# mct10/Speech-Vecalign

Hardware: AMD Instinct MI355X
Metric: aligned doc-pairs/sec (higher is better)
Workload: dtype bf16; 1 GPU; synthetic 4096x4096 d=1024 bf16 embeddings, 4 overlap layers/side, 10 alignment types, band 14, coarse-to-fine (max_size_full_dp=300), 1024 doc-pairs per GPU per step; pipeline=1, N=4096, M=4096, d=1024, overlaps=4, parallelism=dp1 (pairs sharded, no collective)

## Files before the change

### include/svx.h

```cpp
#ifndef SVX_H
#define SVX_H

#include <stdint.h>

#ifdef __cplusplus
extern "C" {
#endif

typedef struct svx_ctx svx_ctx;

enum svx_dtype { SVX_F32 = 0, SVX_F16 = 1, SVX_BF16 = 2 };

enum svx_status {
    SVX_OK = 0,
    SVX_ERR_ARG = 1,
    SVX_ERR_OVERLAPS = 2,
    SVX_ERR_HIP = 3,
    SVX_ERR_TRACEBACK = 4,
    SVX_ERR_NOMEM = 5,
    SVX_ERR_EXTEND = 6,
    SVX_ERR_PATH = 7,
    SVX_ERR_BP = 8
};

// ... 11 lines not shown


int svx_dense_costs(svx_ctx *ctx, const float *vecs0, int k0, int s0, const float *vecs1, int k1, int s1, int d,
                    const float *norm0, const float *norm1, int offset0, int offset1, float *costs);

int svx_dense_dp(svx_ctx *ctx, const float *cost, int s0, int s1, float pen, double *csum, int32_t *bp);

int svx_score_path(svx_ctx *ctx, const int32_t *xx, const int32_t *yy, int64_t n, const float *norm1,
                   const float *norm2, const float *vecs1, int rows1, const float *vecs2, int rows2, int d, float *out);

int svx_sparse_costs(svx_ctx *ctx, const float *vecs0, int k0, int xsize, const float *vecs1, int k1, int ysize,
                     int d, const float *norms0, const float *norms1, const int32_t *path, int A,
                     const int32_t *types_host, int T, int width_over2, float *costs, int32_t *b_offset);

int svx_sparse_dp(svx_ctx *ctx, const float *costs, const int32_t *b_offset_in, int A, int B,
                  const int32_t *types_host, int T, double del_penalty, int x_in_size, int y_in_size,
                  double *csum, int32_t *xp, int32_t *yp, int32_t *b_offset_out);


int svx_make_norm1(svx_ctx *ctx, float *vecs, int64_t rows, int d);

int svx_downsample(svx_ctx *ctx, const float *vecs, int k, int n, int d, float *half);

int svx_compute_norms(svx_ctx *ctx, const float *vecs0, int k0, int n0, const float *vecs1, int k1, int n1, int d,
                      const int32_t *idx, int samples_per_overlap, float *norms0);

int svx_del_penalty(svx_ctx *ctx, const float *scores, int64_t n, double frac, double *del_penalty);

int svx_dense_traceback(svx_ctx *ctx, const int32_t *bp, int s0, int s1, int32_t *align, int32_t *count);

int svx_sparse_traceback(svx_ctx *ctx, const double *csum, const int32_t *xp, const int32_t *yp,
                         const int32_t *b_offset_out, int a_out, int B, int xsize, int ysize, int32_t *align,
                         double *scores, int32_t *count);

int svx_search_path(svx_ctx *ctx, const int32_t *align, const int32_t *n_align, int upsample, int size0,
                    int size1, int32_t *path, int32_t *path_len);

int svx_gather_rows(svx_ctx *ctx, const void *table, int64_t n_rows, int d, int dtype, const int32_t *idx, int64_t n_out,
                    void *out);


int svx_mt19937_choice(uint32_t *key, int32_t *pos, int64_t n, int64_t size, int32_t *out);

int64_t svx_norm_index_count(int n, int m, int k0, int k1, int max_size_full_dp, int num_samps_for_norm, int have_norms0,
                             int have_norms1);
int64_t svx_knob_index_count(int n, int m, int max_size_full_dp, int costs_sample_size);

int svx_draw_indices(uint32_t *key, int32_t *pos, int n, int m, int k0, int k1, int max_size_full_dp, int costs_sample_size,
                     int num_samps_for_norm, int have_norms0, int have_norms1, int32_t *norm_idx, int32_t *knob_idx);

int svx_candidate_table(const char *seg_path, const char *cat_path, const char *ignore_path, int max_overlaps, int32_t *table,
                        int cap_lines, int32_t *n_lines, int64_t *n_candidates, char *err, int err_cap);

int64_t svx_format_alignments(const int32_t *rows, const double *scores, int64_t n, char *out, int64_t cap);


#define SVX_MARGIN_RATIO 0
#define SVX_MARGIN_DISTANCE 1
#define SVX_MARGIN_ABSOLUTE 2

int svx_unit_rows(svx_ctx *ctx, const void *rows, int dtype, int64_t n, int d, void *out, int out_dtype);

int svx_knn_mean_sim(svx_ctx *ctx, const void *queries, int q_dtype, int64_t n, const void *db, int db_dtype,
                     int64_t n_db, int d, int k, float *mean_sim);

int svx_knn_topk_merge(svx_ctx *ctx, const void *queries, int q_dtype, int64_t n, const void *db, int db_dtype,
// ... 130 lines not shown
```

### speech-vecalign_amd/csrc/svx_api.hip

```cpp
#include <stdarg.h>
#include <stdio.h>
#include <stdlib.h>
#include <string.h>

#include <chrono>
#include <functional>
#include <memory>
#include <type_traits>
#include <vector>

#include "svx_common.h"

static char g_err[512] = "";

int svx_fail(svx_ctx* ctx, int code, const char* fmt, ...) {
    char* dst = ctx ? ctx->err : g_err;
    va_list ap;
    va_start(ap, fmt);
    vsnprintf(dst, 512, fmt, ap);
    va_end(ap);
    return code;
}

static const char* kStageNames[] = {"pyr0",       "pyrN",     "pyr_aux",      "knob_scoresN", "knob",      "dense_costs",
// ... 435 lines not shown
    float* part = reinterpret_cast<float*>(ctx->arena + o_part);
    float* mean = reinterpret_cast<float*>(ctx->arena + o_mean);
    if ((rc = svxl_pairsum(ctx, vecs, k, n, d, half, part, nblk))) return rc;
    if ((rc = svxl_colmean_plain(ctx, part, k, nblk, d, h, mean))) return rc;
    return svxl_sub_mean(ctx, half, k, h, d, mean);
}

int svx_compute_norms(svx_ctx* ctx, const float* vecs0, int k0, int n0, const float* vecs1, int k1, int n1, int d,
                      const int32_t* idx, int samples_per_overlap, float* norms0) {
    NEED(ctx, ctx && vecs0 && vecs1 && idx && norms0, "svx_compute_norms: null argument");
    NEED(ctx, n1 > 0 && samples_per_overlap > 0 && k1 > 0, "svx_compute_norms: nothing to sample");
    int rc = check_dim(ctx, d);
    if (rc) return rc;
    rc = arena_reserve(ctx, (size_t)d * sizeof(float) + 256);
    if (rc) return rc;
    float* rbar = reinterpret_cast<float*>(ctx->arena);
    if ((rc = svxl_sample_mean_plain(ctx, vecs1, k1, n1, d, idx, samples_per_overlap, rbar))) return rc;
    return svxl_norms_from_rbar(ctx, vecs0, (int64_t)k0 * n0, d, rbar, norms0);
}

int svx_del_penalty(svx_ctx* ctx, const float* scores, int64_t n, double frac, double* del_penalty) {
    NEED(ctx, ctx && scores && del_penalty && n > 0, "svx_del_penalty: null/empty argument");
    return svxl_del_penalty(ctx, scores, n, frac, del_penalty);
}

int svx_dense_traceback(svx_ctx* ctx, const int32_t* bp, int s0, int s1, int32_t* align, int32_t* count) {
    NEED(ctx, ctx && bp && align && count, "svx_dense_traceback: null argument");
    return svxl_dense_traceback(ctx, bp, s0, s1, align, count);
}

int svx_sparse_traceback(svx_ctx* ctx, const double* csum, const int32_t* xp, const int32_t* yp, const int32_t* b_offset_out,
                         int a_out, int B, int xsize, int ysize, int32_t* align, double* scores, int32_t* count) {
    NEED(ctx, ctx && csum && xp && yp && b_offset_out && align && scores && count, "svx_sparse_traceback: null argument");
    return svxl_sparse_traceback(ctx, csum, xp, yp, b_offset_out, a_out, B, xsize, ysize, align, scores, count);
}

int svx_search_path(svx_ctx* ctx, const int32_t* align, const int32_t* n_align, int upsample, int size0, int size1,
                    int32_t* path, int32_t* path_len) {
    NEED(ctx, ctx && align && n_align && path && path_len, "svx_search_path: null argument");
    return svxl_search_path(ctx, align, n_align, upsample, size0, size1, path, size0 + size1 + 4, path_len);
}

int svx_gather_rows(svx_ctx* ctx, const void* table, int64_t n_rows, int d, int dtype, const int32_t* idx, int64_t n_out, void* out) {
    NEED(ctx, ctx && table && idx && out, "svx_gather_rows: null argument");
    NEED(ctx, dtype == SVX_F32 || dtype == SVX_F16 || dtype == SVX_BF16, "svx_gather_rows: unknown dtype %d", dtype);
    int rc = check_dim(ctx, d);
    if (rc) return rc;
    return svxl_gather_rows(ctx, table, n_rows, d * (dtype == SVX_F32 ? 4 : 2), dtype, idx, n_out, out);
}

}

__global__ void k_init_batch(const SvxPairDev* pairs) {
    const SvxPairDev& P = pairs[blockIdx.x];
    if (threadIdx.x != 0) return;
    *P.status = 0;
    for (int l = 0; l <= P.L; l++) {
        if (P.lev[l].n_align) *P.lev[l].n_align = 0;
        if (P.lev[l].path_len) *P.lev[l].path_len = 0;
    }
    if (P.straight) {
        int* r = P.lev[0].align;
        r[0] = 0; r[1] = P.lev[0].n[0]; r[2] = 0; r[3] = P.lev[0].n[1];
        *P.lev[0].n_align = 1;
    }
}

// ... 421 lines not shown
    cur.lb.push_back({(np * (H.maxL + 1) * 0.21 < 300.0 ? 300.0 : np * (H.maxL + 1) * 0.21), S_KNOB,
                      [=]() { return svxl_del_penalty_batch(ctx, h->dpairs, np, h->maxL + 1, bp.frac); }});
    if (!bp.straight)
        cur.lb.push_back({(H.max_ds0 + H.max_ds1) * 1.7 * waves, S_DENSE_DP, [=]() { return svxl_dense_stage_batch(ctx, h->dpairs, np, h->max_ds0); }});
    const int first_depth = H.maxL > 0 ? H.maxL - 1 : 0;
    for (int depth = first_depth; depth >= 0; depth--) {
        const SvxTypes ty = depth == 0 ? bp.tfinal : bp.t11;
        int lim2 = 0, tamax2 = 0;
        const bool v2 = !bp.tiles && svxl_band2_limits(ty, W, depth, dtype, d, &lim2, &tamax2);
        const int maxA = H.max_A[depth];
        const int src_rows = (H.maxL > 0 && !H.any_L0) ? maxA / 2 + 8 : maxA;
        cur.lb.push_back({maxA * 0.08 * waves + 60.0, depth == 0 ? S_PATH0 : S_PATH, [=]() {
            return svxl_search_path_batch(ctx, h->dpairs, np, depth, maxA, src_rows, v2 ? lim2 : SVX_BC_ROWS - SVX_BC_TB,
                                          bp.tiles ? 0 : (v2 ? tamax2 : SVX_BC_TAMAX));
        }});
        cur.has_s = true;
        if (bp.tiles) {
            cur.s = {1.0e4, S_TILES, [=]() {
                int* tk = reinterpret_cast<int*>(h->arena + h->o_tickets);
                float* planes = h->b_planes ? reinterpret_cast<float*>(h->arena + h->o_planes) : nullptr;
                return svxl_band_tiles_batch(ctx, h->dpairs, np, ty, W, dtype, h->max_tnd, tk, tk + (size_t)h->max_tnd * np + 1, planes);
            }};
        } else {
            cur.s = {H.b_bc[depth] / 4.0e6, depth == 0 ? S_BAND_COSTS0 : S_BAND_COSTSN, [=]() {
                return v2 ? svxl_band_costs2_batch(ctx, h->dpairs, np, depth, maxA, ty, W, dtype, d)
                          : svxl_band_costs_batch(ctx, h->dpairs, np, depth, maxA, ty, W, dtype, d);
            }};
        }
        segs.push_back(cur);
        cur = Seg();
        if (!bp.tiles)
            cur.lb.push_back({maxA * (0.21 + 0.054 * (ty.n > 1 ? ty.n : 0)) * waves, depth == 0 ? S_BAND_DP0 : S_BAND_DPN,
                              [=]() { return svxl_sparse_dp_batch(ctx, h->dpairs, np, depth, ty, B); }});
        cur.lb.push_back({maxA * 0.27 * waves, depth == 0 ? S_TRACEBACK0 : S_TRACEBACK, [=]() { return svxl_sparse_traceback_batch(ctx, h->dpairs, np, depth, B, maxA, bp.packable ? 1 : 0); }});
    }
    segs.push_back(cur);
}

static int ensure_streams(svx_ctx* ctx) {
    svx_ctx_ext* cx = X(ctx);
    if (!cx->side_ready) {
        int prio_lo = 0, prio_hi = 0;
        SVX_HIP(ctx, hipDeviceGetStreamPriorityRange(&prio_lo, &prio_hi));
        SVX_HIP(ctx, hipStreamCreateWithPriority(&cx->side, hipStreamNonBlocking, prio_lo));
        SVX_HIP(ctx, hipStreamCreateWithPriority(&cx->helper, hipStreamNonBlocking, prio_hi));
        SVX_HIP(ctx, hipEventCreateWithFlags(&cx->side_fork, hipEventDisableTiming));
        SVX_HIP(ctx, hipEventCreateWithFlags(&cx->side_join, hipEventDisableTiming));
        cx->side_ready = true;
    }
    if (!cx->chain_ready) {
        int prio_lo = 0, prio_hi = 0;
        SVX_HIP(ctx, hipDeviceGetStreamPriorityRange(&prio_lo, &prio_hi));
        SVX_HIP(ctx, hipStreamCreateWithPriority(&cx->chain, hipStreamNonBlocking, prio_hi));
        cx->chain_ready = true;
    }
    for (int h = 0; h < 2; h++) {
        if (!cx->half[h].front_done) SVX_HIP(ctx, hipEventCreateWithFlags(&cx->half[h].front_done, hipEventDisableTiming));
        if (!cx->half[h].chain_done) SVX_HIP(ctx, hipEventCreateWithFlags(&cx->half[h].chain_done, hipEventDisableTiming));
        if (!cx->half[h].upload_done) SVX_HIP(ctx, hipEventCreateWithFlags(&cx->half[h].upload_done, hipEventDisableTiming));
    }
    return SVX_OK;
}

static int run_interleaved(svx_ctx* ctx, HalfState* front, HalfState* chain, bool beside) {
    svx_ctx_ext* cx = X(ctx);
    hipStream_t A = ctx->stream, Bst = beside ? cx->chain : ctx->stream;
    std::vector<Op> fops;
// ... 204 lines not shown
```

### speech-vecalign_amd/csrc/svx_common.h

```cpp
#pragma once
#include <hip/hip_runtime.h>
#include <stdint.h>
#include <stddef.h>
#include "../../include/svx.h"

#define SVX_WAVE 64

#ifndef SVX_PYR_SLOTS
#define SVX_PYR_SLOTS 32
#endif
#define SVX_BC_TA 32
#define SVX_BC_TAMAX 64
#define SVX_BC_TB 16
#define SVX_BC_ROWS 48

struct ElemF32 {
    using storage = float;
    static constexpr int VEC = 4;
    static constexpr int DT = SVX_F32;
};
struct ElemF16 {
    using storage = uint16_t;
    static constexpr int VEC = 8;
    static constexpr int DT = SVX_F16;
// ... 234 lines not shown
int svxl_sub_mean(svx_ctx*, float* half, int k, int h, int d, const float* mean);
int svxl_sample_mean_plain(svx_ctx*, const float* vecs, int k, int n, int d, const int* idx, int S, float* rbar);
int svxl_norms_from_rbar(svx_ctx*, const float* vecs, int64_t rows, int d, const float* rbar, float* norms);
int svxl_gather_rows(svx_ctx*, const void* table, long long n_rows, int row_bytes, int dtype, const int* idx, long long n_out, void* out);
int svxl_pyramid_level(svx_ctx*, const SvxPairDev* pairs, int n_pairs, int level, int dtype, int d, int max_nblk,
                       int max_ksum, int part);
int svxl_score_path(svx_ctx*, const int* xx, const int* yy, int64_t n, const float* n1, const float* n2,
                    const float* v1, int rows1, const float* v2, int rows2, int d, float* out);
int svxl_knob_scores(svx_ctx*, const SvxPairDev* pairs, int n_pairs, int max_levels, int max_kn, int max_n0, int dtype, int d,
                     int part);
int svxl_dense_costs(svx_ctx*, const float* v0, int s0, const float* v1, int s1, int d, const float* n0,
                     const float* n1, int mul0, int mul1, float* costs);
int svxl_dense_costs_batch(svx_ctx*, const SvxPairDev* pairs, int n_pairs, int max_s0, int max_s1, int dtype, int d);
int svxl_knob_from_dots(svx_ctx*, const SvxPairDev* pairs, int n_pairs, int max_kn);
int svxl_band_costs(svx_ctx*, const void* v0, int k0, int n, const void* v1, int k1, int m, int d, int dtype,
                    const float* inv0, const float* inv1, const float* nrm0, const float* nrm1, const int* path,
                    int A, const SvxTypes& types, int W, float* costs, int* boff, int* status);
int svxl_band_costs_batch(svx_ctx*, const SvxPairDev* pairs, int n_pairs, int depth, int max_A, const SvxTypes& types,
                          int W, int dtype, int d);
bool svxl_band2_limits(const SvxTypes& types, int W, int depth, int dtype, int d, int* lim, int* tamax);
int svxl_band_costs2_batch(svx_ctx*, const SvxPairDev* pairs, int n_pairs, int depth, int max_A, const SvxTypes& types, int W,
                           int dtype, int d);
int svxl_band_tiles_shape(const SvxTypes& types);
size_t svxl_band_tiles_scratch(const SvxTypes& types);
int svxl_band_tiles_batch(svx_ctx*, const SvxPairDev* pairs, int n_pairs, const SvxTypes& types, int W, int dtype, int max_nd,
                          int* gpref, int* ticket, float* planes);
int svxl_dense_dp(svx_ctx*, const float* cost, int s0, int s1, float pen, double* csum, int* bp);
int svxl_dense_stage_batch(svx_ctx*, const SvxPairDev* pairs, int n_pairs, int max_s0);
int svxl_dense_traceback(svx_ctx*, const int* bp, int s0, int s1, int* align, int* count);
int svxl_sparse_dp(svx_ctx*, const float* costs, const int* boff_in, int A, int B, const SvxTypes& types, double pen,
                   int xs, int ys, double* csum, int* xp, int* yp, int* boff_out);
int svxl_sparse_dp_batch(svx_ctx*, const SvxPairDev* pairs, int n_pairs, int depth, const SvxTypes& types, int B);
int svxl_sparse_traceback(svx_ctx*, const double* csum, const int* xp, const int* yp, const int* boff, int a_out,
                          int B, int xs, int ys, int* align, double* scores, int* count);
int svxl_sparse_traceback_batch(svx_ctx*, const SvxPairDev* pairs, int n_pairs, int depth, int B, int max_A, int packed);
int svxl_search_path(svx_ctx*, const int* align, const int* n_align, int upsample, int size0, int size1, int* path,
                     int cap, int* path_len);
int svxl_search_path_batch(svx_ctx*, const SvxPairDev* pairs, int n_pairs, int depth, int max_rows, int max_src_rows, int chunk_lim,
                           int chunk_tamax);
int svxl_del_penalty(svx_ctx*, const float* scores, int64_t n, double frac, double* out);
int svxl_del_penalty_batch(svx_ctx*, const SvxPairDev* pairs, int n_pairs, int max_levels, double frac);
int svxl_prior_ingest_batch(svx_ctx*, const SvxPairDev* pairs, int n_pairs);
bool svxl_last_batch(svx_ctx*, const SvxPairDev** host, int* n_pairs, int* band);
```

### speech-vecalign_amd/csrc/svx_dp.hip

```cpp
#include <stdlib.h>

#include "svx_common.h"

namespace {

struct DenseDpArgs {
    const float* cost;
    int s0, s1;
    float pen;
    double* csum;
    int* bp;
    int diag;
};

__device__ void dense_dp_block(const DenseDpArgs& g, double* ring) {
    const int rmax = g.s0 + 1, cmax = g.s1 + 1;
    const int tid = threadIdx.x, nt = blockDim.x;
    const double pen_d = (double)g.pen;
    auto cost_of = [&](int k, int r) -> float {
        const int c = k - r;
        return (r >= 1 && r <= g.s0 && c >= 1 && c <= g.s1) ? g.cost[(size_t)(r - 1) * g.s1 + (c - 1)] : 0.f;
    };
    float cnext = cost_of(0, tid);
    for (int k = 0; k <= g.s0 + g.s1; k++) {
// ... 531 lines not shown
}

template <bool RING>
__global__ __launch_bounds__(1024) void k_sparse_dp_batch(const SvxPairDev* __restrict__ pairs, int depth, SvxTypes ty, int B) {
    extern __shared__ __attribute__((aligned(16))) char smem[];
    SparseDpArgs g;
    if (!batch_dp_args(pairs[blockIdx.x], depth, B, &g)) return;
    const size_t ring_bytes = RING ? (((size_t)(ty.maxstep + 1) * g.B * sizeof(double) + 15) & ~(size_t)15) : 0;
    sparse_dp_block<RING>(g, ty, reinterpret_cast<double*>(smem), reinterpret_cast<int*>(smem + ring_bytes));
}

template <int TPLT, int G>
__global__ __launch_bounds__(DPF_THREADS) void k_sparse_dp_fast_batch(const SvxPairDev* __restrict__ pairs, int depth,
                                                                       SvxTypes ty, int B, int CH) {
    extern __shared__ __attribute__((aligned(16))) char smem[];
    SparseDpArgs g;
    if (!batch_dp_args(pairs[blockIdx.x], depth, B, &g)) return;
    sparse_dp_fast<TPLT, G>(g, ty, CH, smem);
}

struct TbArgs {
    const double* csum;
    const int* xp;
    const int* yp;
    const unsigned char* bpk;
    const int* boff;
    int Aout, B, xs, ys;
    int* align;
    double* scores;
    int* count;
    int* status;
    int chunk;
    int cw;
};

__host__ __device__ inline size_t tb_win_bytes(int chunk, int B, bool wide) {
    const size_t bp = (size_t)chunk * B * (wide ? 2 : 1);
    return ((bp + 15) & ~(size_t)15) + (size_t)chunk * sizeof(int);
}
constexpr int TB_COR_CHUNK = 64, TB_COR_W = 320;
__host__ __device__ inline size_t tb_smem_bytes(int chunk, int B, bool wide) { return 2 * tb_win_bytes(chunk, B, wide); }
__host__ __device__ inline int tb_chunk(int B, bool wide, int win_kb = 20) {
    const int c = (int)(((size_t)win_kb * 1024) / ((size_t)B * (wide ? 2 : 1) + sizeof(int))) & ~15;
    if (c >= 64) return c;
    const int c20 = (int)((20 * 1024) / ((size_t)B * (wide ? 2 : 1) + sizeof(int))) & ~15;
    return c20 >= 64 ? c20 : 0;
}
static int tb_win_kb() {
    static const int v = [] { const char* e = getenv("SVX_TB_WIN_KB"); const int k = e ? atoi(e) : 20; return k >= 2 && k <= 64 ? k : 20; }();
    return v;
}

__device__ __forceinline__ void tb_load_corridor(const TbArgs& g, char* win, int j, int c0, int tsub, int nsub) {
    const int lo = j * g.chunk;
    const int hi = (lo + g.chunk) < g.Aout ? (lo + g.chunk) : g.Aout;
    int* lbo = reinterpret_cast<int*>(win + ((((size_t)g.chunk * g.cw) + 15) & ~(size_t)15));
    for (int i = tsub; i < hi - lo; i += nsub) lbo[i] = g.boff[lo + i];
    const int ppr = g.cw / 16;
    const int n = (hi - lo) * ppr;
    for (int e = tsub; e < n; e += nsub) {
        const int i = e / ppr, p = e - i * ppr;
        reinterpret_cast<uint4*>(win)[e] = *reinterpret_cast<const uint4*>(g.bpk + (size_t)(lo + i) * g.B + c0 + 16 * p);
    }
}

__device__ __forceinline__ void tb_load_window(const TbArgs& g, char* win, int j, int tsub, int nsub) {
    const int B = g.B, lo = j * g.chunk;
    const int hi = (lo + g.chunk) < g.Aout ? (lo + g.chunk) : g.Aout;
    const bool wide = g.bpk == nullptr;
    int* lbo = reinterpret_cast<int*>(win + ((((size_t)g.chunk * B * (wide ? 2 : 1)) + 15) & ~(size_t)15));
    for (int i = tsub; i < hi - lo; i += nsub) lbo[i] = g.boff[lo + i];
    const size_t first = (size_t)lo * B, nb = (size_t)(hi - lo) * B;
    if (!wide) {
        unsigned char* lbp = reinterpret_cast<unsigned char*>(win);
        const unsigned char* src = g.bpk + first;
        if ((reinterpret_cast<size_t>(src) & 15) == 0) {
            const size_t nv = nb / 16;
            for (size_t i = tsub; i < nv; i += nsub) reinterpret_cast<uint4*>(lbp)[i] = reinterpret_cast<const uint4*>(src)[i];
            for (size_t i = nv * 16 + tsub; i < nb; i += nsub) lbp[i] = src[i];
        } else {
            for (size_t i = tsub; i < nb; i += nsub) lbp[i] = src[i];
        }
// ... 45 lines not shown
            py = v == 0xFFFF ? -42 : (v & 255);
        } else {
            const size_t o = (size_t)aa * B + bb;
            if (g.bpk) {
                const int v = __builtin_amdgcn_readfirstlane((int)g.bpk[o]);
                px = v == 0xFF ? -42 : (v >> 4);
                py = v == 0xFF ? -42 : (v & 15);
            } else {
                px = __builtin_amdgcn_readfirstlane(g.xp[o]);
                py = __builtin_amdgcn_readfirstlane(g.yp[o]);
            }
        }
        if (px < 0 || py < 0 || (px == 0 && py == 0) || px > xx || py > yy) { err = SVX_ERR_TRACEBACK; break; }
        const int ln = nw & 63;
        {
            const bool me = (int)threadIdx.x == ln;
            r0 = me ? xx - px : r0;
            r1 = me ? px : r1;
            r2 = me ? yy - py : r2;
            r3 = me ? py : r3;
        }
        xx -= px;
        yy -= py;
        nw++;
        if ((nw & 63) == 0) {
            flush(first_pending, nw);
            first_pending = nw;
        }
    }
    nw = __builtin_amdgcn_readfirstlane(nw);
    if (first_pending < nw) flush(first_pending, nw);
}

__device__ void sparse_traceback_block(const TbArgs& g, char* smem) {
    __shared__ int sh_n;
    __shared__ int sh_c0[2];
    const int cap = g.xs + g.ys + 2;
    const int Aout = g.Aout, B = g.B;
    const bool wide = g.bpk == nullptr;
    const bool cor = g.cw > 0;
    if (Aout < 1 || B < 1 || g.xs < 0 || g.ys < 0) {
        if (threadIdx.x == 0) {
            *g.count = -SVX_ERR_TRACEBACK;
            if (g.status) *g.status = SVX_ERR_TRACEBACK;
        }
        return;
    }
    const size_t win_bytes = g.chunk > 0 ? (cor ? tb_win_bytes(g.chunk, g.cw, false) : tb_win_bytes(g.chunk, B, wide)) : 0;
    const int nwin = g.chunk > 0 ? (Aout + g.chunk - 1) / g.chunk : 1;
    int xx = __builtin_amdgcn_readfirstlane(g.xs), yy = __builtin_amdgcn_readfirstlane(g.ys), nw = 0, err = 0;
    const bool wave0 = __builtin_amdgcn_readfirstlane((int)(threadIdx.x >> 6)) == 0;
    bool done = false;
    if (g.chunk > 0) {
        if (cor) {
            const int aa = g.xs + g.ys;
            const int b_end = (aa >= 0 && aa < Aout) ? g.ys - g.boff[aa] : 0;
            if (threadIdx.x == 0) {
                int c = (b_end - g.cw / 2) & ~15;
                c = c < 0 ? 0 : (c > B - g.cw ? B - g.cw : c);
                sh_c0[(nwin - 1) & 1] = c;
            }
            __syncthreads();
            tb_load_corridor(g, smem + (size_t)((nwin - 1) & 1) * win_bytes, nwin - 1, sh_c0[(nwin - 1) & 1], threadIdx.x, blockDim.x);
        } else {
            tb_load_window(g, smem + (size_t)((nwin - 1) & 1) * win_bytes, nwin - 1, threadIdx.x, blockDim.x);
        }
        __syncthreads();
    }
    for (int j = nwin - 1; j >= 0; j--) {
        if (cor && j > 0) {
            if (threadIdx.x == 0) {
                const int aa = xx + yy;
                const int bnow = (aa >= 0 && aa < Aout) ? yy - g.boff[aa] : 0;
                int c = (bnow - g.cw / 2) & ~15;
                c = c < 0 ? 0 : (c > B - g.cw ? B - g.cw : c);
                sh_c0[(j - 1) & 1] = c;
            }
            __syncthreads();
            if (threadIdx.x >= 64) tb_load_corridor(g, smem + (size_t)((j - 1) & 1) * win_bytes, j - 1, sh_c0[(j - 1) & 1], threadIdx.x - 64, blockDim.x - 64);
        } else if (g.chunk > 0 && j > 0 && threadIdx.x >= 64) tb_load_window(g, smem + (size_t)((j - 1) & 1) * win_bytes, j - 1, threadIdx.x - 64, blockDim.x - 64);
        if (wave0 && !done && !err) {
            const int lo = g.chunk > 0 ? j * g.chunk : 0;
            const char* win = smem + (size_t)(j & 1) * win_bytes;
            const unsigned char* lbp = reinterpret_cast<const unsigned char*>(win);
            const unsigned short* lbw = reinterpret_cast<const unsigned short*>(win);
            const int* lbo = reinterpret_cast<const int*>(win + ((((size_t)g.chunk * (cor ? g.cw : B) * ((wide && !cor) ? 2 : 1)) + 15) & ~(size_t)15));
            const int c0w = cor ? __builtin_amdgcn_readfirstlane(sh_c0[j & 1]) : 0;
            if (cor) tb_walk<3>(g, lbp, lbw, lbo, lo, c0w, cap, xx, yy, nw, err, done);
            else if (g.chunk > 0 && !wide) tb_walk<1>(g, lbp, lbw, lbo, lo, c0w, cap, xx, yy, nw, err, done);
            else if (g.chunk > 0) tb_walk<2>(g, lbp, lbw, lbo, lo, c0w, cap, xx, yy, nw, err, done);
            else tb_walk<0>(g, lbp, lbw, lbo, lo, c0w, cap, xx, yy, nw, err, done);
        }
        if (g.chunk > 0) __syncthreads();
    }
    if (threadIdx.x == 0) {
        if (!err && !done) err = SVX_ERR_TRACEBACK;

        if (!err) {
            const int aa = g.xs + g.ys;
            const int bb = (aa >= 0 && aa < Aout) ? g.ys - g.boff[aa] : -1;
            if (bb < 0 || bb >= B) err = SVX_ERR_TRACEBACK;
        }
// ... 15 lines not shown
    const int nt = blockDim.x;
    for (int base = 0; base < n; base += nt) {
        const int j = base + threadIdx.x;
        int r0 = 0, r1 = 0, r2 = 0, r3 = 0;
        double s = 0.0;
        if (j < n) {
            const int* r = g.align + 4 * (size_t)(cap - n + j);
            r0 = r[0]; r1 = r[1]; r2 = r[2]; r3 = r[3];
            const int xa = r0, ya = r2, xb = r0 + r1, yb = r2 + r3;
            const double c0 = g.csum[(size_t)(xa + ya) * B + (ya - g.boff[xa + ya])];
            const double c1 = g.csum[(size_t)(xb + yb) * B + (yb - g.boff[xb + yb])];
            const double cost = c1 - c0;
            s = cost < 0.0 ? 0.0 : cost;
            if (r1 == 0 || r3 == 0) s = 0.0;
            else s = s / (double)r1 / (double)r3;
        }
        __syncthreads();
        if (j < n) {
            int* w = g.align + 4 * (size_t)j;
            w[0] = r0; w[1] = r1; w[2] = r2; w[3] = r3;
            g.scores[j] = s;
        }
        __syncthreads();
    }
    if (threadIdx.x == 0) *g.count = n;
}

__global__ __launch_bounds__(256) void k_sparse_traceback(TbArgs g) {
    extern __shared__ __attribute__((aligned(16))) char smem[];
    sparse_traceback_block(g, smem);
}

__global__ __launch_bounds__(256) void k_sparse_traceback_batch(const SvxPairDev* __restrict__ pairs, int depth, int B,
                                                                int chunk, int cw) {
    extern __shared__ __attribute__((aligned(16))) char smem[];
    const SvxPairDev& P = pairs[blockIdx.x];
    if (depth > P.L || (depth == P.L && P.L > 0)) return;
    if (*P.status != 0) return;
    const SvxLevel& Lv = P.lev[depth];
    const int A = *Lv.path_len;
    if (A <= 0) return;
    TbArgs g;
    g.csum = Lv.csum; g.xp = Lv.xp; g.yp = Lv.yp; g.bpk = Lv.bpk; g.boff = Lv.boff_out;
    g.Aout = A + 2; g.B = B; g.xs = Lv.n[0]; g.ys = Lv.n[1];
    g.align = Lv.align; g.scores = Lv.scores; g.count = Lv.n_align; g.status = P.status;
    g.chunk = chunk;
    g.cw = cw;
    sparse_traceback_block(g, smem);
}

__device__ int slant(int* path, int n, int cap, int xw, int yw, int& lx, int& ly) {
    const int NN = xw + yw;
    const int xs = lx, ys = ly;
    for (int ii = 1; ii <= NN; ii++) {
        const int x = xs + (int)rint((double)((long long)xw * ii) / (double)NN);
        const int y = ys + (int)rint((double)((long long)yw * ii) / (double)NN);
        const int delta = x + y - lx - ly;
        int nx, ny;
        if (delta == 1) { nx = x; ny = y; }
        else if (delta == 2) { nx = x - 1; ny = y; }
        else if (delta == 0) { nx = x + 1; ny = y; }
        else continue;
        if (n >= cap) return -SVX_ERR_PATH;
        *reinterpret_cast<int2*>(path + 2 * (size_t)n) = make_int2(nx, ny);
        lx = nx;
        ly = ny;
        n++;
    }
    return n;
}

__device__ int search_path_thread(const int* align, int n_align, int upsample, int size0, int size1, int* path, int cap) {
    if (cap < 1) return -SVX_ERR_PATH;
    int n = 1, xdel = 0, ydel = 0;
    const int f = upsample ? 2 : 1;
    int xmax = 0, ymax = 0;
    int lx = 0, ly = 0;
    path[0] = 0;
    path[1] = 0;
    for (int i = 0; i < n_align; i++) {
// ... 398 lines not shown
    do {                                                                                                              \
        if (G == 4) DPF_LAUNCH(TPLT, 4); else if (G == 2) DPF_LAUNCH(TPLT, 2); else DPF_LAUNCH(TPLT, 1);               \
    } while (0)
        const int G = dpf_groups(types.n, B);
        switch (dpf_tpl(types.n, B)) {
            case 1: DPF_LAUNCH_G(1); break;
            case 2: DPF_LAUNCH_G(2); break;
            case 3: DPF_LAUNCH_G(3); break;
            case 4: DPF_LAUNCH_G(4); break;
            case 6: DPF_LAUNCH_G(6); break;
            default: DPF_LAUNCH_G(0); break;
        }
#undef DPF_LAUNCH_G
#undef DPF_LAUNCH
        SVX_LAUNCH_CHECK(ctx, "k_sparse_dp_fast_batch");
        return SVX_OK;
    }
    const size_t ring = (((size_t)(types.maxstep + 1) * B * sizeof(double)) + 15) & ~(size_t)15;
    const size_t tabs = wide_tab_bytes(types.n + 2);
    const int nt = dp_threads(B);
    if (ring + tabs <= 150 * 1024) {
        const size_t smem = ring + tabs;
        if (smem > 64 * 1024)
            SVX_HIP(ctx, hipFuncSetAttribute((const void*)k_sparse_dp_batch<true>, hipFuncAttributeMaxDynamicSharedMemorySize, (int)smem));
        hipLaunchKernelGGL(k_sparse_dp_batch<true>, dim3(n_pairs), dim3(nt), smem, ctx->stream, pairs, depth, types, B);
    } else {
        hipLaunchKernelGGL(k_sparse_dp_batch<false>, dim3(n_pairs), dim3(nt), tabs, ctx->stream, pairs, depth, types, B);
    }
    SVX_LAUNCH_CHECK(ctx, "k_sparse_dp_batch");
    return SVX_OK;
}


int svxl_sparse_traceback(svx_ctx* ctx, const double* csum, const int* xp, const int* yp, const int* boff, int a_out, int B,
                          int xs, int ys, int* align, double* scores, int* count) {
    TbArgs g;
    g.csum = csum; g.xp = xp; g.yp = yp; g.bpk = nullptr; g.boff = boff;
    g.Aout = a_out; g.B = B; g.xs = xs; g.ys = ys;
    g.align = align; g.scores = scores; g.count = count; g.status = nullptr;
    g.chunk = tb_chunk(B, true, tb_win_kb());
    g.cw = 0;
    const size_t smem = g.chunk > 0 ? tb_smem_bytes(g.chunk, B, true) : 0;
    if (smem > 64 * 1024)
        SVX_HIP(ctx, hipFuncSetAttribute((const void*)k_sparse_traceback, hipFuncAttributeMaxDynamicSharedMemorySize, (int)smem));
    hipLaunchKernelGGL(k_sparse_traceback, dim3(1), dim3(256), smem, ctx->stream, g);
    SVX_LAUNCH_CHECK(ctx, "k_sparse_traceback");
    return SVX_OK;
}

int svxl_sparse_traceback_batch(svx_ctx* ctx, const SvxPairDev* pairs, int n_pairs, int depth, int B, int max_A, int packed) {
    if (n_pairs <= 0) return SVX_OK;
    int chunk = tb_chunk(B, !packed, tb_win_kb()), cw = 0;
    size_t smem = chunk > 0 ? tb_smem_bytes(chunk, B, !packed) : 0;
    if (chunk == 0 && packed && B > TB_COR_W && B % 16 == 0) {
        chunk = TB_COR_CHUNK;
        cw = TB_COR_W;
        smem = 2 * tb_win_bytes(chunk, cw, false);
    }
    (void)max_A;
    if (smem > 64 * 1024)
        SVX_HIP(ctx, hipFuncSetAttribute((const void*)k_sparse_traceback_batch, hipFuncAttributeMaxDynamicSharedMemorySize, (int)smem));
    hipLaunchKernelGGL(k_sparse_traceback_batch, dim3(n_pairs), dim3(256), smem, ctx->stream, pairs, depth, B, chunk, cw);
    SVX_LAUNCH_CHECK(ctx, "k_sparse_traceback_batch");
    return SVX_OK;
}

static const size_t SP_LDS_LIMIT = 150 * 1024;

static int sp_lds_rows(int max_rows, size_t* smem) {
    int rows = max_rows;
    if (sp_smem_bytes(rows) > SP_LDS_LIMIT) rows = (int)(SP_LDS_LIMIT / (4 * sizeof(int))) - 3;
    *smem = sp_smem_bytes(rows);
    return rows;
}

int svxl_search_path(svx_ctx* ctx, const int* align, const int* n_align, int upsample, int size0, int size1, int* path,
                     int cap, int* path_len) {
    size_t smem;
    const int rows = sp_lds_rows(size0 + size1 + 2, &smem);
    if (smem > 64 * 1024)
        SVX_HIP(ctx, hipFuncSetAttribute((const void*)k_search_path, hipFuncAttributeMaxDynamicSharedMemorySize, (int)smem));
    hipLaunchKernelGGL(k_search_path, dim3(1), dim3(256), smem, ctx->stream, align, n_align, upsample, size0, size1, path, cap,
                       path_len, rows);
    SVX_LAUNCH_CHECK(ctx, "k_search_path");
    return SVX_OK;
}

int svxl_search_path_batch(svx_ctx* ctx, const SvxPairDev* pairs, int n_pairs, int depth, int max_rows, int max_src_rows, int chunk_lim,
                           int chunk_tamax) {
    if (n_pairs <= 0) return SVX_OK;
    size_t smem;
    const int rows = sp_lds_rows(max_src_rows, &smem);
    if (smem > 64 * 1024)
        SVX_HIP(ctx, hipFuncSetAttribute((const void*)k_search_path_batch, hipFuncAttributeMaxDynamicSharedMemorySize, (int)smem));
    hipLaunchKernelGGL(k_search_path_batch, dim3(n_pairs), dim3(256), smem, ctx->stream, pairs, depth, rows);
// ... 25 lines not shown
```

### speech-vecalign_amd/svx/_lib.py

```python
import ctypes
import os
import threading

_HERE = os.path.dirname(os.path.abspath(__file__))
LIB_PATH = os.environ.get("SVX_LIB") or os.path.join(_HERE, "libsvx.so")

SVX_F32, SVX_F16, SVX_BF16 = 0, 1, 2
SVX_MAX_TYPES = 128
SVX_MAX_LEVELS = 16
SVX_MARGIN_RATIO, SVX_MARGIN_DISTANCE, SVX_MARGIN_ABSOLUTE = 0, 1, 2
SVX_SEARCH_COARSE_TO_FINE, SVX_SEARCH_STRAIGHT, SVX_SEARCH_AROUND, SVX_SEARCH_AROUND_WIDE = 0, 1, 2, 3

SVX_OK, SVX_ERR_ARG, SVX_ERR_OVERLAPS, SVX_ERR_HIP, SVX_ERR_TRACEBACK = 0, 1, 2, 3, 4
SVX_ERR_NOMEM, SVX_ERR_EXTEND, SVX_ERR_PATH, SVX_ERR_BP = 5, 6, 7, 8

DEVICE_ERRORS = {
    SVX_ERR_TRACEBACK: "traceback bug",
    SVX_ERR_BP: "got unknown value",
    SVX_ERR_EXTEND: "asked to extend alignments but already bigger than requested",
    SVX_ERR_PATH: "search path is not a unit-step lattice path",
}

c_int, c_i64, c_f32, c_f64, c_vp = ctypes.c_int, ctypes.c_int64, ctypes.c_float, ctypes.c_double, ctypes.c_void_p

# ... 52 lines not shown
class ConcatParams(ctypes.Structure):
    _fields_ = [
        ("max_score", ctypes.c_double),
        ("max_num_align", ctypes.c_int32), ("sample_rate", ctypes.c_int32),
        ("max_sil", ctypes.c_double), ("max_dur", ctypes.c_double),
        ("both_sides", ctypes.c_int32), ("pad", ctypes.c_int32),
        ("min_frames", ctypes.c_int64),
    ]


SVX_CONCAT_MAX = 8

_SIGS = {
    "svx_create": (c_int, [c_int, ctypes.POINTER(c_vp)]),
    "svx_destroy": (c_int, [c_vp]),
    "svx_set_stream": (c_int, [c_vp, c_vp]),
    "svx_synchronize": (c_int, [c_vp]),
    "svx_last_error": (ctypes.c_char_p, [c_vp]),
    "svx_version": (ctypes.c_char_p, []),
    "svx_scratch_bytes": (c_i64, [c_vp]),
    "svx_dense_costs": (c_int, [c_vp, c_vp, c_int, c_int, c_vp, c_int, c_int, c_int, c_vp, c_vp, c_int, c_int, c_vp]),
    "svx_dense_dp": (c_int, [c_vp, c_vp, c_int, c_int, c_f32, c_vp, c_vp]),
    "svx_score_path": (c_int, [c_vp, c_vp, c_vp, c_i64, c_vp, c_vp, c_vp, c_int, c_vp, c_int, c_int, c_vp]),
    "svx_sparse_costs": (c_int, [c_vp, c_vp, c_int, c_int, c_vp, c_int, c_int, c_int, c_vp, c_vp, c_vp, c_int,
                                 ctypes.POINTER(ctypes.c_int32), c_int, c_int, c_vp, c_vp]),
    "svx_sparse_dp": (c_int, [c_vp, c_vp, c_vp, c_int, c_int, ctypes.POINTER(ctypes.c_int32), c_int, c_f64, c_int, c_int,
                              c_vp, c_vp, c_vp, c_vp]),
    "svx_make_norm1": (c_int, [c_vp, c_vp, c_i64, c_int]),
    "svx_downsample": (c_int, [c_vp, c_vp, c_int, c_int, c_int, c_vp]),
    "svx_compute_norms": (c_int, [c_vp, c_vp, c_int, c_int, c_vp, c_int, c_int, c_int, c_vp, c_int, c_vp]),
    "svx_del_penalty": (c_int, [c_vp, c_vp, c_i64, c_f64, c_vp]),
    "svx_dense_traceback": (c_int, [c_vp, c_vp, c_int, c_int, c_vp, c_vp]),
    "svx_sparse_traceback": (c_int, [c_vp, c_vp, c_vp, c_vp, c_vp, c_int, c_int, c_int, c_int, c_vp, c_vp, c_vp]),
    "svx_search_path": (c_int, [c_vp, c_vp, c_vp, c_int, c_int, c_int, c_vp, c_vp]),
    "svx_gather_rows": (c_int, [c_vp, c_vp, c_i64, c_int, c_int, c_vp, c_i64, c_vp]),
    "svx_unit_rows": (c_int, [c_vp, c_vp, c_int, c_i64, c_int, c_vp, c_int]),
    "svx_knn_mean_sim": (c_int, [c_vp, c_vp, c_int, c_i64, c_vp, c_int, c_i64, c_int, c_int, c_vp]),
    "svx_knn_topk_merge": (c_int, [c_vp, c_vp, c_int, c_i64, c_vp, c_int, c_i64, c_int, c_int, c_vp, c_int, c_vp]),
    "svx_knn_search": (c_int, [c_vp, c_vp, c_int, c_i64, c_vp, c_int, c_i64, c_int, c_int, c_i64, c_vp, c_vp, c_int]),
    "svx_knn_search_groups": (c_int, [c_vp, c_vp, c_int, c_vp, c_int, c_int, c_int, c_vp, c_vp, c_int, c_vp, c_vp]),
    "svx_margin_scores": (c_int, [c_vp, c_vp, c_vp, c_int, c_i64, c_int, c_vp, c_vp, c_int, c_vp]),
    "svx_knn_list_means": (c_int, [c_vp, c_vp, c_i64, c_int, c_vp]),
    "svx_margin_candidates": (c_int, [c_vp, c_vp, c_vp, c_i64, c_int, c_vp, c_vp, c_i64, c_i64, c_int, c_vp, c_vp, c_vp]),
    "svx_mine_greedy": (c_i64, [c_vp, c_i64, c_vp, c_vp, c_i64, c_i64, c_vp]),
    "svx_mt19937_choice": (c_int, [c_vp, ctypes.POINTER(ctypes.c_int32), c_i64, c_i64, c_vp]),
    "svx_norm_index_count": (c_i64, [c_int, c_int, c_int, c_int, c_int, c_int, c_int, c_int]),
    "svx_knob_index_count": (c_i64, [c_int, c_int, c_int, c_int]),
    "svx_draw_indices": (c_int, [c_vp, ctypes.POINTER(ctypes.c_int32), c_int, c_int, c_int, c_int, c_int, c_int, c_int, c_int, c_int,
                                 c_vp, c_vp]),
    "svx_candidate_table": (c_int, [ctypes.c_char_p, ctypes.c_char_p, ctypes.c_char_p, c_int, c_vp, c_int,
                                    ctypes.POINTER(ctypes.c_int32), ctypes.POINTER(c_i64), ctypes.c_char_p, c_int]),
    "svx_format_alignments": (c_i64, [c_vp, c_vp, c_i64, c_vp, c_i64]),
    "svx_num_levels": (c_int, [c_int, c_int, c_int]),
    "svx_knob_count": (c_i64, [c_int, c_int, c_int]),
    "svx_align_batch": (c_int, [c_vp, ctypes.POINTER(AlignParams), ctypes.POINTER(Pair), c_int]),
    "svx_align_around": (c_int, [c_vp, ctypes.POINTER(AlignParams), ctypes.POINTER(Pair), ctypes.POINTER(Prior), c_int]),
    "svx_time_prior": (c_int, [c_vp, ctypes.POINTER(Pair), ctypes.POINTER(Frames), c_int, c_i64, c_i64, ctypes.POINTER(Prior)]),
    "svx_prior_width": (c_int, [c_vp, ctypes.POINTER(Pair), ctypes.POINTER(Prior), c_int, c_vp]),
    "svx_band_contact": (c_int, [c_vp, c_int, c_int, c_vp]),
    "svx_align_widen": (c_int, [c_vp, ctypes.POINTER(AlignParams), ctypes.POINTER(Pair), ctypes.POINTER(Prior), c_int,
                                ctypes.POINTER(WidenParams), c_vp]),
    "svx_alignment_rows": (c_int, [c_vp, c_int, c_int, ctypes.POINTER(Pair), c_int, c_f64, c_i64, c_vp, c_vp, c_vp, c_vp, c_int, c_vp, c_vp]),
    "svx_concat_rows": (c_int, [c_vp, c_int, c_int, ctypes.POINTER(Pair), ctypes.POINTER(Frames), c_int, ctypes.POINTER(ConcatParams), c_i64,
                                c_vp, c_vp, c_vp, c_vp, c_int, c_vp, c_vp]),
    "svx_debug_level": (c_int, [c_vp, c_int, c_int, ctypes.POINTER(LevelView)]),
    "svx_copy_to_host": (c_int, [c_vp, c_vp, c_vp, c_i64]),
# ... 111 lines not shown
```

Measured before the change: 9585 doc-pairs/s.

## Parallelize sparse traceback with per-segment jump tables and parallel emit

Replaces the serial backpointer walk within each shared-memory window with a parallel scheme. Threads precompute, for every 64-diagonal segment and entry offset, where the path exits, then one thread stitches the segments and the threads write the alignment rows in parallel. It falls back to the serial walk when a step exceeds max_step. It also updates the scheduler cost estimate for traceback and adds an _ex API that can pack backpointers to bytes. The cost is extra shared memory and redundant table work for entries the path never visits.

```diff
diff --git a/include/svx.h b/include/svx.h
--- a/include/svx.h
+++ b/include/svx.h
@@ -67,6 +67,10 @@
 int svx_sparse_traceback(svx_ctx *ctx, const double *csum, const int32_t *xp, const int32_t *yp,
                          const int32_t *b_offset_out, int a_out, int B, int xsize, int ysize, int32_t *align,
                          double *scores, int32_t *count);
+
+int svx_sparse_traceback_ex(svx_ctx *ctx, const double *csum, const int32_t *xp, const int32_t *yp,
+                            const int32_t *b_offset_out, int a_out, int B, int xsize, int ysize, int32_t *align,
+                            double *scores, int32_t *count, int max_step);
 
 int svx_search_path(svx_ctx *ctx, const int32_t *align, const int32_t *n_align, int upsample, int size0,
                     int size1, int32_t *path, int32_t *path_len);
diff --git a/speech-vecalign_amd/csrc/svx_api.hip b/speech-vecalign_amd/csrc/svx_api.hip
--- a/speech-vecalign_amd/csrc/svx_api.hip
+++ b/speech-vecalign_amd/csrc/svx_api.hip
@@ -491,7 +491,14 @@
 int svx_sparse_traceback(svx_ctx* ctx, const double* csum, const int32_t* xp, const int32_t* yp, const int32_t* b_offset_out,
                          int a_out, int B, int xsize, int ysize, int32_t* align, double* scores, int32_t* count) {
     NEED(ctx, ctx && csum && xp && yp && b_offset_out && align && scores && count, "svx_sparse_traceback: null argument");
-    return svxl_sparse_traceback(ctx, csum, xp, yp, b_offset_out, a_out, B, xsize, ysize, align, scores, count);
+    return svxl_sparse_traceback(ctx, csum, xp, yp, b_offset_out, a_out, B, xsize, ysize, align, scores, count, 0);
+}
+
+int svx_sparse_traceback_ex(svx_ctx* ctx, const double* csum, const int32_t* xp, const int32_t* yp, const int32_t* b_offset_out,
+                            int a_out, int B, int xsize, int ysize, int32_t* align, double* scores, int32_t* count, int max_step) {
+    NEED(ctx, ctx && csum && xp && yp && b_offset_out && align && scores && count, "svx_sparse_traceback_ex: null argument");
+    NEED(ctx, max_step >= -30 && max_step <= 200, "svx_sparse_traceback_ex: max_step must be in [-30, 200]");
+    return svxl_sparse_traceback(ctx, csum, xp, yp, b_offset_out, a_out, B, xsize, ysize, align, scores, count, max_step);
 }
 
 int svx_search_path(svx_ctx* ctx, const int32_t* align, const int32_t* n_align, int upsample, int size0, int size1,
@@ -979,7 +986,7 @@
         if (!bp.tiles)
             cur.lb.push_back({maxA * (0.21 + 0.054 * (ty.n > 1 ? ty.n : 0)) * waves, depth == 0 ? S_BAND_DP0 : S_BAND_DPN,
                               [=]() { return svxl_sparse_dp_batch(ctx, h->dpairs, np, depth, ty, B); }});
-        cur.lb.push_back({maxA * 0.27 * waves, depth == 0 ? S_TRACEBACK0 : S_TRACEBACK, [=]() { return svxl_sparse_traceback_batch(ctx, h->dpairs, np, depth, B, maxA, bp.packable ? 1 : 0); }});
+        cur.lb.push_back({maxA * svxl_traceback_us_per_diag(B, bp.packable ? 1 : 0, ty.maxstep) * waves, depth == 0 ? S_TRACEBACK0 : S_TRACEBACK, [=]() { return svxl_sparse_traceback_batch(ctx, h->dpairs, np, depth, B, maxA, bp.packable ? 1 : 0, ty.maxstep); }});
     }
     segs.push_back(cur);
 }
diff --git a/speech-vecalign_amd/csrc/svx_common.h b/speech-vecalign_amd/csrc/svx_common.h
--- a/speech-vecalign_amd/csrc/svx_common.h
+++ b/speech-vecalign_amd/csrc/svx_common.h
@@ -290,8 +290,9 @@
                    int xs, int ys, double* csum, int* xp, int* yp, int* boff_out);
 int svxl_sparse_dp_batch(svx_ctx*, const SvxPairDev* pairs, int n_pairs, int depth, const SvxTypes& types, int B);
 int svxl_sparse_traceback(svx_ctx*, const double* csum, const int* xp, const int* yp, const int* boff, int a_out,
-                          int B, int xs, int ys, int* align, double* scores, int* count);
-int svxl_sparse_traceback_batch(svx_ctx*, const SvxPairDev* pairs, int n_pairs, int depth, int B, int max_A, int packed);
+                          int B, int xs, int ys, int* align, double* scores, int* count, int max_step);
+int svxl_sparse_traceback_batch(svx_ctx*, const SvxPairDev* pairs, int n_pairs, int depth, int B, int max_A, int packed, int max_step);
+double svxl_traceback_us_per_diag(int B, int packed, int max_step);
 int svxl_search_path(svx_ctx*, const int* align, const int* n_align, int upsample, int size0, int size1, int* path,
                      int cap, int* path_len);
 int svxl_search_path_batch(svx_ctx*, const SvxPairDev* pairs, int n_pairs, int depth, int max_rows, int max_src_rows, int chunk_lim,
diff --git a/speech-vecalign_amd/csrc/svx_dp.hip b/speech-vecalign_amd/csrc/svx_dp.hip
--- a/speech-vecalign_amd/csrc/svx_dp.hip
+++ b/speech-vecalign_amd/csrc/svx_dp.hip
@@ -587,6 +587,8 @@
     int* status;
     int chunk;
     int cw;
+    int max_step;
+    int nps;
 };
 
 __host__ __device__ inline size_t tb_win_bytes(int chunk, int B, bool wide) {
@@ -603,6 +605,27 @@
 }
 static int tb_win_kb() {
     static const int v = [] { const char* e = getenv("SVX_TB_WIN_KB"); const int k = e ? atoi(e) : 20; return k >= 2 && k <= 64 ? k : 20; }();
+    return v;
+}
+
+constexpr int TB_SEG = 64;
+constexpr int TB_MAXSEG = 64;
+constexpr int TB_TBL_MAX = 1792;
+enum { TBX_EXIT = 0, TBX_ORIGIN = 1, TBX_DEAD = 2, TBX_OVER = 3 };
+__host__ __device__ inline int tb_par_segs(int chunk, int B, int max_step, int cw) {
+    if (max_step <= 0 || chunk <= 0 || cw > 0 || 2 * max_step > TB_SEG) return 0;
+    const long long per = (long long)max_step * B;
+    if (2 * per > TB_TBL_MAX) return 0;
+    int n = (int)(TB_TBL_MAX / per);
+    const int need = (chunk + TB_SEG - 1) / TB_SEG;
+    n = n < need ? n : need;
+    n = n < TB_MAXSEG ? n : TB_MAXSEG;
+    return n >= 2 ? n : 0;
+}
+__host__ __device__ inline size_t tb_par_tbl_bytes(int nps, int B, int max_step) { return (((size_t)nps * max_step * B * sizeof(unsigned)) + 15) & ~(size_t)15; }
+__host__ __device__ inline size_t tb_par_bytes(int nps, int B, int max_step) { return nps > 0 ? tb_par_tbl_bytes(nps, B, max_step) + (size_t)nps * 16 : 0; }
+static bool tb_serial() {
+    static const bool v = [] { const char* e = getenv("SVX_TB_SERIAL"); return e && atoi(e) != 0; }();
     return v;
 }
 
@@ -714,9 +737,148 @@
     if (first_pending < nw) flush(first_pending, nw);
 }
 
+template <int MODE>
+__device__ __forceinline__ bool tb_bp(const unsigned char* lbp, const unsigned short* lbw, size_t o, int& px, int& py) {
+    if (MODE == 1) {
+        const int v = lbp[o];
+        px = v >> 4; py = v & 15;
+        return v != 0xFF;
+    }
+    const int v = lbw[o];
+    px = v >> 8; py = v & 255;
+    return v != 0xFFFF;
+}
+
+template <int MODE>
+__device__ __forceinline__ void tb_par_table(const TbArgs& g, const unsigned char* lbp, const unsigned short* lbw, const int* lbo, int lo,
+                                             int top, int nseg, unsigned* tbl) {
+    const int B = g.B, ms = g.max_step, per = ms * B, n = nseg * per;
+    for (int e = threadIdx.x; e < n; e += blockDim.x) {
+        const int k = e / per, r = e - k * per, d = r / B, b0 = r - d * B;
+        const int segtop = top - k * TB_SEG;
+        const int seglo = segtop - TB_SEG + 1 > lo ? segtop - TB_SEG + 1 : lo;
+        unsigned code = TBX_DEAD;
+        int rows = 0, dx = 0, dy = 0;
+        int aa = segtop - d;
+        if (aa >= seglo) {
+            int yy = (int)((unsigned)b0 + (unsigned)lbo[aa - lo]);
+            int xx = (int)((unsigned)aa - (unsigned)yy);
+            if (xx >= 0 && yy >= 0) {
+                for (int t = 0; t <= TB_SEG; t++) {
+                    if (xx == 0 && yy == 0) { code = TBX_ORIGIN; break; }
+                    aa = xx + yy;
+                    if (aa < seglo) { code = TBX_EXIT; break; }
+                    const int bb = (int)((unsigned)yy - (unsigned)lbo[aa - lo]);
+                    if (bb < 0 || bb >= B) break;
+                    int px, py;
+                    if (!tb_bp<MODE>(lbp, lbw, (size_t)(aa - lo) * B + bb, px, py)) break;
+                    if ((px | py) == 0 || px > xx || py > yy) break;
+                    if (px + py > ms) { code = TBX_OVER; break; }
+                    xx -= px; yy -= py;
+                    dx += px; dy += py;
+                    rows++;
+                }
+            }
+        }
+        tbl[e] = code << 30 | (unsigned)rows << 16 | (unsigned)dx << 8 | (unsigned)dy;
+    }
+}
+
+__device__ __forceinline__ void tb_par_stitch(const TbArgs& g, const int* lbo, int lo, int top, int nseg, int cap, const unsigned* tbl,
+                                              int4* sent, int* st) {
+    const int B = g.B, ms = g.max_step;
+    int xx = st[0], yy = st[1], nw = st[2], err = 0, done = 0, fb = 0, k = 0;
+    for (; k < nseg; k++) {
+        if (xx == 0 && yy == 0) { done = 1; break; }
+        const int aa = xx + yy;
+        if (aa < lo) break;
+        const int d = top - k * TB_SEG - aa;
+        if (d < 0 || d >= ms) { fb = 1; break; }
+        const int bb = (int)((unsigned)yy - (unsigned)lbo[aa - lo]);
+        if (nw >= cap - 1 || bb < 0 || bb >= B) { err = SVX_ERR_TRACEBACK; break; }
+        const unsigned t = tbl[(k * ms + d) * B + bb];
+        const unsigned code = t >> 30;
+        const int rows = (int)((t >> 16) & 127);
+        if (code == TBX_OVER) { fb = 1; break; }
+        if (code == TBX_DEAD || nw + rows > cap - 1) { err = SVX_ERR_TRACEBACK; break; }
+        sent[k] = make_int4(xx, yy, nw, rows);
+        xx -= (int)((t >> 8) & 255);
+        yy -= (int)(t & 255);
+        nw += rows;
+        if (code == TBX_ORIGIN) { done = 1; k++; break; }
+    }
+    st[5] = fb;
+    st[6] = k;
+    if (!fb) { st[0] = xx; st[1] = yy; st[2] = nw; st[3] = err; st[4] = done; }
+}
+
+template <int MODE>
+__device__ __forceinline__ void tb_par_emit(const TbArgs& g, const unsigned char* lbp, const unsigned short* lbw, const int* lbo, int lo,
+                                            int cap, const int4* sent, int nemit) {
+    const int k = (int)(threadIdx.x & 63) * 4 + (int)(threadIdx.x >> 6);
+    if (k >= nemit) return;
+    const int4 s = sent[k];
+    int xx = s.x, yy = s.y, idx = s.z;
+    for (int t = 0; t < s.w; t++) {
+        const int aa = xx + yy;
+        const int bb = (int)((unsigned)yy - (unsigned)lbo[aa - lo]);
+        int px, py;
+        (void)tb_bp<MODE>(lbp, lbw, (size_t)(aa - lo) * g.B + bb, px, py);
+        gst16(g.align + 4 * (size_t)(cap - 1 - idx), (uint32_t)(xx - px), (uint32_t)px, (uint32_t)(yy - py), (uint32_t)py);
+        xx -= px; yy -= py;
+        idx++;
+    }
+}
+
+template <int MODE>
+__device__ __forceinline__ void tb_par_window(const TbArgs& g, const char* win, int lo, int cap, unsigned* tbl, int4* sent, int* st) {
+    const int Aout = g.Aout, B = g.B;
+    const unsigned char* lbp = reinterpret_cast<const unsigned char*>(win);
+    const unsigned short* lbw = reinterpret_cast<const unsigned short*>(win);
+    const int* lbo = reinterpret_cast<const int*>(win + ((((size_t)g.chunk * B * (MODE == 2 ? 2 : 1)) + 15) & ~(size_t)15));
+    const bool wave0 = __builtin_amdgcn_readfirstlane((int)(threadIdx.x >> 6)) == 0;
+    const int max_pass = g.chunk / TB_SEG + 2;
+    for (int pass = 0; pass < max_pass; pass++) {
+        __syncthreads();
+        if (st[3] != 0 || st[4] != 0) return;
+        const int top = st[0] + st[1];
+        if (top < lo) return;
+        if (top >= lo + g.chunk) break;
+        int nseg = 0;
+        if (top < Aout) {
+            nseg = (top - lo) / TB_SEG + 1;
+            nseg = nseg < g.nps ? nseg : g.nps;
+        }
+        if (nseg >= 2) {
+            tb_par_table<MODE>(g, lbp, lbw, lbo, lo, top, nseg, tbl);
+            __syncthreads();
+            if (threadIdx.x == 0) tb_par_stitch(g, lbo, lo, top, nseg, cap, tbl, sent, st);
+            __syncthreads();
+            if (st[5] == 0) {
+                if (st[3] == 0) tb_par_emit<MODE>(g, lbp, lbw, lbo, lo, cap, sent, st[6]);
+                continue;
+            }
+        }
+        int xx = st[0], yy = st[1], nw = st[2], err = 0;
+        bool done = false;
+        __syncthreads();
+        if (wave0) {
+            xx = __builtin_amdgcn_readfirstlane(xx);
+            yy = __builtin_amdgcn_readfirstlane(yy);
+            nw = __builtin_amdgcn_readfirstlane(nw);
+            tb_walk<MODE>(g, lbp, lbw, lbo, lo, 0, cap, xx, yy, nw, err, done);
+            if (threadIdx.x == 0) { st[0] = xx; st[1] = yy; st[2] = nw; st[3] = err; st[4] = done ? 1 : 0; }
+        }
+        return;
+    }
+    __syncthreads();
+    if (threadIdx.x == 0) st[3] = SVX_ERR_TRACEBACK;
+}
+
 __device__ void sparse_traceback_block(const TbArgs& g, char* smem) {
     __shared__ int sh_n;
     __shared__ int sh_c0[2];
+    __shared__ int sh_st[8];
     const int cap = g.xs + g.ys + 2;
     const int Aout = g.Aout, B = g.B;
     const bool wide = g.bpk == nullptr;
@@ -749,7 +911,19 @@
         }
         __syncthreads();
     }
-    for (int j = nwin - 1; j >= 0; j--) {
+    if (g.nps > 0) {
+        unsigned* tbl = reinterpret_cast<unsigned*>(smem + 2 * win_bytes);
+        int4* sent = reinterpret_cast<int4*>(smem + 2 * win_bytes + tb_par_tbl_bytes(g.nps, B, g.max_step));
+        if (threadIdx.x == 0) { sh_st[0] = g.xs; sh_st[1] = g.ys; sh_st[2] = 0; sh_st[3] = 0; sh_st[4] = 0; }
+        for (int j = nwin - 1; j >= 0; j--) {
+            if (j > 0) tb_load_window(g, smem + (size_t)((j - 1) & 1) * win_bytes, j - 1, threadIdx.x, blockDim.x);
+            const char* win = smem + (size_t)(j & 1) * win_bytes;
+            if (wide) tb_par_window<2>(g, win, j * g.chunk, cap, tbl, sent, sh_st);
+            else tb_par_window<1>(g, win, j * g.chunk, cap, tbl, sent, sh_st);
+            __syncthreads();
+        }
+        xx = sh_st[0]; yy = sh_st[1]; nw = sh_st[2]; err = sh_st[3]; done = sh_st[4] != 0;
+    } else for (int j = nwin - 1; j >= 0; j--) {
         if (cor && j > 0) {
             if (threadIdx.x == 0) {
                 const int aa = xx + yy;
@@ -831,7 +1005,7 @@
 }
 
 __global__ __launch_bounds__(256) void k_sparse_traceback_batch(const SvxPairDev* __restrict__ pairs, int depth, int B,
-                                                                int chunk, int cw) {
+                                                                int chunk, int cw, int max_step, int nps) {
     extern __shared__ __attribute__((aligned(16))) char smem[];
     const SvxPairDev& P = pairs[blockIdx.x];
     if (depth > P.L || (depth == P.L && P.L > 0)) return;
@@ -845,6 +1019,8 @@
     g.align = Lv.align; g.scores = Lv.scores; g.count = Lv.n_align; g.status = P.status;
     g.chunk = chunk;
     g.cw = cw;
+    g.max_step = max_step;
+    g.nps = nps;
     sparse_traceback_block(g, smem);
 }
 
@@ -1309,23 +1485,55 @@
 }
 
 
+__global__ void k_tb_pack(const int* __restrict__ xp, const int* __restrict__ yp, size_t n, unsigned char* __restrict__ bpk) {
+    for (size_t i = (size_t)blockIdx.x * blockDim.x + threadIdx.x; i < n; i += (size_t)gridDim.x * blockDim.x) {
+        const int px = xp[i], py = yp[i];
+        bpk[i] = (px < 0 || py < 0 || px > 15 || py > 15) ? (unsigned char)0xFF : (unsigned char)((px << 4) | py);
+    }
+}
+
 int svxl_sparse_traceback(svx_ctx* ctx, const double* csum, const int* xp, const int* yp, const int* boff, int a_out, int B,
-                          int xs, int ys, int* align, double* scores, int* count) {
+                          int xs, int ys, int* align, double* scores, int* count, int max_step) {
+    const bool pack = max_step < 0 && a_out >= 1 && B >= 1;
     TbArgs g;
     g.csum = csum; g.xp = xp; g.yp = yp; g.bpk = nullptr; g.boff = boff;
     g.Aout = a_out; g.B = B; g.xs = xs; g.ys = ys;
     g.align = align; g.scores = scores; g.count = count; g.status = nullptr;
-    g.chunk = tb_chunk(B, true, tb_win_kb());
+    g.chunk = tb_chunk(B, !pack, tb_win_kb());
     g.cw = 0;
-    const size_t smem = g.chunk > 0 ? tb_smem_bytes(g.chunk, B, true) : 0;
-    if (smem > 64 * 1024)
-        SVX_HIP(ctx, hipFuncSetAttribute((const void*)k_sparse_traceback, hipFuncAttributeMaxDynamicSharedMemorySize, (int)smem));
-    hipLaunchKernelGGL(k_sparse_traceback, dim3(1), dim3(256), smem, ctx->stream, g);
-    SVX_LAUNCH_CHECK(ctx, "k_sparse_traceback");
+    g.max_step = tb_serial() ? 0 : (max_step < 0 ? -max_step : max_step);
+    g.nps = tb_par_segs(g.chunk, B, g.max_step, 0);
+    unsigned char* bpk = nullptr;
+    if (pack) {
+        const size_t n = (size_t)a_out * B;
+        SVX_HIP(ctx, hipMalloc(reinterpret_cast<void**>(&bpk), n));
+        hipLaunchKernelGGL(k_tb_pack, dim3((unsigned)((n + 255) / 256 < 1024 ? (n + 255) / 256 : 1024)), dim3(256), 0, ctx->stream, xp, yp, n, bpk);
+        g.bpk = bpk;
+        g.xp = g.yp = nullptr;
+    }
+    const size_t smem = g.chunk > 0 ? tb_smem_bytes(g.chunk, B, !pack) + tb_par_bytes(g.nps, B, g.max_step) : 0;
+    hipError_t e = hipSuccess;
+    if (smem > 64 * 1024) e = hipFuncSetAttribute((const void*)k_sparse_traceback, hipFuncAttributeMaxDynamicSharedMemorySize, (int)smem);
+    if (e == hipSuccess) {
+        hipLaunchKernelGGL(k_sparse_traceback, dim3(1), dim3(256), smem, ctx->stream, g);
+        e = hipGetLastError();
+    }
+    if (bpk) {
+        const hipError_t es = hipStreamSynchronize(ctx->stream);
+        (void)hipFree(bpk);
+        if (e == hipSuccess) e = es;
+    }
+    SVX_HIP(ctx, e);
     return SVX_OK;
 }
 
-int svxl_sparse_traceback_batch(svx_ctx* ctx, const SvxPairDev* pairs, int n_pairs, int depth, int B, int max_A, int packed) {
+double svxl_traceback_us_per_diag(int B, int packed, int max_step) {
+    const int chunk = tb_chunk(B, !packed, tb_win_kb());
+    if (tb_serial() || tb_par_segs(chunk, B, max_step, 0) == 0) return 0.27;
+    return max_step <= 2 ? 0.09 : 0.13;
+}
+
+int svxl_sparse_traceback_batch(svx_ctx* ctx, const SvxPairDev* pairs, int n_pairs, int depth, int B, int max_A, int packed, int max_step) {
     if (n_pairs <= 0) return SVX_OK;
     int chunk = tb_chunk(B, !packed, tb_win_kb()), cw = 0;
     size_t smem = chunk > 0 ? tb_smem_bytes(chunk, B, !packed) : 0;
@@ -1335,9 +1543,12 @@
         smem = 2 * tb_win_bytes(chunk, cw, false);
     }
     (void)max_A;
+    if (tb_serial()) max_step = 0;
+    const int nps = tb_par_segs(chunk, B, max_step, cw);
+    smem += tb_par_bytes(nps, B, max_step);
     if (smem > 64 * 1024)
         SVX_HIP(ctx, hipFuncSetAttribute((const void*)k_sparse_traceback_batch, hipFuncAttributeMaxDynamicSharedMemorySize, (int)smem));
-    hipLaunchKernelGGL(k_sparse_traceback_batch, dim3(n_pairs), dim3(256), smem, ctx->stream, pairs, depth, B, chunk, cw);
+    hipLaunchKernelGGL(k_sparse_traceback_batch, dim3(n_pairs), dim3(256), smem, ctx->stream, pairs, depth, B, chunk, cw, max_step, nps);
     SVX_LAUNCH_CHECK(ctx, "k_sparse_traceback_batch");
     return SVX_OK;
 }
diff --git a/speech-vecalign_amd/svx/_lib.py b/speech-vecalign_amd/svx/_lib.py
--- a/speech-vecalign_amd/svx/_lib.py
+++ b/speech-vecalign_amd/svx/_lib.py
@@ -108,6 +108,7 @@
     "svx_del_penalty": (c_int, [c_vp, c_vp, c_i64, c_f64, c_vp]),
     "svx_dense_traceback": (c_int, [c_vp, c_vp, c_int, c_int, c_vp, c_vp]),
     "svx_sparse_traceback": (c_int, [c_vp, c_vp, c_vp, c_vp, c_vp, c_int, c_int, c_int, c_int, c_vp, c_vp, c_vp]),
+    "svx_sparse_traceback_ex": (c_int, [c_vp, c_vp, c_vp, c_vp, c_vp, c_int, c_int, c_int, c_int, c_vp, c_vp, c_vp, c_int]),
     "svx_search_path": (c_int, [c_vp, c_vp, c_vp, c_int, c_int, c_int, c_vp, c_vp]),
     "svx_gather_rows": (c_int, [c_vp, c_vp, c_i64, c_int, c_int, c_vp, c_i64, c_vp]),
     "svx_unit_rows": (c_int, [c_vp, c_vp, c_int, c_i64, c_int, c_vp, c_int]),
```

Result: no change. 9595 doc-pairs/s, median of 2 (+0.1%).
